# Deci-AI/super-gradients

Hardware: NVIDIA H100
Metric: images/sec YOLO-NAS-S 640 bf16 train (higher is better)
Workload: dtype bf16

## Files before the change

include/sgb200.h:

```cpp
#ifndef SGB200_H_
#define SGB200_H_

#include <stdint.h>

#ifdef __cplusplus
extern "C" {
#endif

#define SGB_OK 0
#define SGB_E_INVALID (-1)
#define SGB_E_UNSUPPORTED (-2)
#define SGB_E_CUDA (-3)
#define SGB_E_ARCH (-4)

#define SGB_ACT_NONE 0
#define SGB_ACT_RELU 1
#define SGB_ACT_SILU 2

typedef uint16_t sgb_bf16;

typedef struct SgbConvDesc {
  int32_t N, H, W, C;
  int32_t K, R, S;
  int32_t P, Q;
  int32_t stride, pad;
  int32_t x_pitch, x_off;
  int32_t y_pitch, y_off;
  int32_t up2;
  int32_t centre_from;
} SgbConvDesc;

typedef struct SgbEpilogue {
  const float* scale;
  const float* shift;
  const sgb_bf16* residual;
  double* stats;
  int32_t stats_repl;
  int32_t act;
  int32_t out_f32;
} SgbEpilogue;

const char* sgb_last_error(void);
int sgb_version(void);
int sgb_check_device(void);
int64_t sgb_sm100_launches(void);
int64_t sgb_conv_halo_launches(void);
void sgb_conv_force_im2col(int on);
int64_t sgb_conv_wgrad_halo_launches(void);
void sgb_conv_wgrad_force_im2col(int on);

int sgb_conv_fprop(const SgbConvDesc* d, const sgb_bf16* x, const sgb_bf16* w_krsc, void* y, const SgbEpilogue* ep,
                   void* stream);
int sgb_conv_dgrad(const SgbConvDesc* d, const sgb_bf16* dy, const sgb_bf16* w_crsk, sgb_bf16* dx, int accumulate,
                   void* stream);
int sgb_conv_wgrad(const SgbConvDesc* d, const sgb_bf16* x, const sgb_bf16* dy, float* dw_krsc, void* stream);
int sgb_weight_prepare(const float* w_oihw, int K, int C, int R, int S, int c_pad, sgb_bf16* w_krsc, sgb_bf16* w_crsk,
                       const float* scale, int add_identity, void* stream);
int sgb_wgrad_to_oihw(const float* dw_krsc, int K, int C, int R, int S, int c_pad, float* g_oihw, int accumulate,
                      void* stream);
typedef struct SgbWeightItem {
  const float* w;
  const float* scale;
  sgb_bf16* krsc;
  sgb_bf16* crsk;
  int32_t K, C, R, S, c_pad, add_identity;
  int32_t kp, koff, etaps, etap;
  int64_t start;
} SgbWeightItem;
typedef struct SgbWgradItem {
  const float* dw;
  float* g;
  int32_t K, C, R, S, c_pad, accumulate;
  int64_t start;
} SgbWgradItem;
int sgb_weight_prepare_batch(const SgbWeightItem* items_dev, int n_items, int64_t total, void* stream);
typedef struct SgbAlphaItem {
  const float* dw1;
  const float* w1;
  const float* alpha;
// ... 348 lines not shown
```

super_gradients_b200/csrc/capi.cu:

```cuda
#include <cstdarg>
#include <cstdio>

#include "common.cuh"
#include "conv_sm100.h"
#include "sm100_host.h"

static thread_local char g_err[512] = "";

void sgb_set_error(const char* fmt, ...) {
  va_list ap;
  va_start(ap, fmt);
  vsnprintf(g_err, sizeof(g_err), fmt, ap);
  va_end(ap);
}

int sgb_cuda_check(cudaError_t e, const char* what) {
  if (e == cudaSuccess) return SGB_OK;
  sgb_set_error("%s: %s", what, cudaGetErrorString(e));
  return SGB_E_CUDA;
}

extern "C" const char* sgb_last_error(void) { return g_err; }
extern "C" int sgb_version(void) { return 100; }
extern "C" int sgb_check_device(void) {
  int dev = 0;
  if (int rc = sgb_cuda_check(cudaGetDevice(&dev), "cudaGetDevice")) return rc;
  cudaDeviceProp prop;
  if (int rc = sgb_cuda_check(cudaGetDeviceProperties(&prop, dev), "cudaGetDeviceProperties")) return rc;
  if (prop.major != 9) {
    sgb_set_error("libsgb200 is built for sm_90a only; device is sm_%d%d", prop.major, prop.minor);
    return SGB_E_ARCH;
  }
  return SGB_OK;
}

extern "C" int64_t sgb_sm100_launches(void) { return (int64_t)sm100::launch_count(); }
extern "C" int64_t sgb_conv_halo_launches(void) { return (int64_t)sm100::halo_launch_count(); }
extern "C" void sgb_conv_force_im2col(int on) { sm100::force_im2col(on != 0); }
extern "C" int64_t sgb_conv_wgrad_halo_launches(void) { return (int64_t)sm100::wgrad_halo_launch_count(); }
extern "C" void sgb_conv_wgrad_force_im2col(int on) { sm100::wgrad_force_im2col(on != 0); }
```

super_gradients_b200/csrc/conv_sm100.cu:

```cuda
#include <cuda.h>

#include <cstdlib>
#include <cstring>

#include "common.cuh"
#include "conv_sm100.h"
#include "sm100_host.h"
#include "sm100_ptx.cuh"

namespace sm100 {

constexpr int BLOCK_M = 128;
constexpr int NUM_THREADS = 384;
constexpr int CONSUMER_THREADS = 256;
constexpr int MAX_STAGES = 8;

struct Params {
  int M;
  int N;
  int C;
  int KC;
  int n_tiles;
  int stages;
  int P, Q;
// ... 13 lines not shown
  int stats_repl;
  int act;
  int centre_n, centre_c;
};

template <int BN>
__device__ __forceinline__ int off_centre_steps(const Params& p, int nt, int steps, int step_ch) {
  if (p.centre_n > 0 && nt * BN >= p.centre_n) return 0;
  if (p.centre_c > 0) return (p.centre_c + step_ch - 1) / step_ch;
  return steps;
}
constexpr int CENTRE_TAP = 4;

__device__ __forceinline__ long long out_row(const Params& p, long long m) {
  if (p.out_mode == 0) return m;
  const int pq = p.P * p.Q;
  const int n = (int)(m / pq);
  const int rem = (int)(m - (long long)n * pq);
  const int j = rem / p.Q, i = rem - j * p.Q;
  return ((long long)n * p.outH + j * p.o_mul + p.oh_add) * p.outW + i * p.o_mul + p.ow_add;
}

__device__ __forceinline__ void consumer_sync() { asm volatile("bar.sync 1, %0;" ::"n"(CONSUMER_THREADS) : "memory"); }
template <int WARPS>
__device__ __forceinline__ void group_sync(int wg) {
  if (WARPS == 8)
    consumer_sync();
  else
    asm volatile("bar.sync %0, 128;" ::"r"(2 + wg) : "memory");
}

constexpr uint32_t CTRL_BAR_BYTES = 16u * MAX_STAGES;

template <int BN, int WARPS = 8>
__device__ __forceinline__ void tile_epilogue(const Params& p, const float (&acc)[BN / 2], const long long (&orow)[2],
                                              const bool (&row_ok)[2], int nt, int wg, int wq, int lane, float* s_part,
                                              float* s_stats) {
  const int n0 = nt * BN;
  const int ncols = min(BN, p.N - n0);
  bf16* yrow[2];
  const bf16* rrow[2];
#pragma unroll
  for (int h = 0; h < 2; ++h) {
    yrow[h] = p.y + orow[h] * p.y_pitch + p.y_off + n0;
    rrow[h] = p.residual ? p.residual + orow[h] * p.y_pitch + p.y_off + n0 : nullptr;
  }
#pragma unroll
  for (int j = 0; j < BN / 8; ++j) {
    const int col = 8 * j + 2 * (lane & 3);
    const bool col_ok = col < ncols;
    float sum0 = 0.f, sum1 = 0.f, sq0 = 0.f, sq1 = 0.f;
#pragma unroll
    for (int h = 0; h < 2; ++h) {
      float v0 = acc[4 * j + 2 * h], v1 = acc[4 * j + 2 * h + 1];
      const bool ok = row_ok[h] && col_ok;
      if (p.scale && col_ok) {
        v0 *= p.scale[n0 + col];
        v1 *= p.scale[n0 + col + 1];
      }
      if (p.shift && col_ok) {
        v0 += p.shift[n0 + col];
        v1 += p.shift[n0 + col + 1];
      }
      if (rrow[h] && ok) {
        const uint32_t rr = *reinterpret_cast<const uint32_t*>(rrow[h] + col);
        v0 += __uint_as_float(rr << 16);
        v1 += __uint_as_float(rr & 0xffff0000u);
      }
      if (p.act != SGB_ACT_NONE) {
        v0 = apply_act(v0, p.act);
        v1 = apply_act(v1, p.act);
      }
      __nv_bfloat162 hh = __floats2bfloat162_rn(v0, v1);
      const uint32_t pk = *reinterpret_cast<uint32_t*>(&hh);
      if (ok) {
        *reinterpret_cast<uint32_t*>(yrow[h] + col) = pk;
        const float lo = __uint_as_float(pk << 16), hi = __uint_as_float(pk & 0xffff0000u);
        sum0 += lo;
        sum1 += hi;
        sq0 = fmaf(lo, lo, sq0);
        sq1 = fmaf(hi, hi, sq1);
      }
    }
    if (p.stats) {
#pragma unroll
      for (int o = 4; o < 32; o <<= 1) {
        sum0 += __shfl_xor_sync(0xffffffffu, sum0, o);
        sum1 += __shfl_xor_sync(0xffffffffu, sum1, o);
        sq0 += __shfl_xor_sync(0xffffffffu, sq0, o);
        sq1 += __shfl_xor_sync(0xffffffffu, sq1, o);
      }
      if (lane < 4) {
        float* part = s_part + (WARPS == 8 ? wg * 4 + wq : wq) * 2 * BN;
        part[col] = sum0;
        part[col + 1] = sum1;
        part[BN + col] = sq0;
        part[BN + col + 1] = sq1;
      }
    }
  }
  if (p.stats) {
    group_sync<WARPS>(wg);
    for (int i = threadIdx.x - 128 - (WARPS == 8 ? 0 : 128 * wg); i < 2 * BN; i += WARPS * 32) {
      const int which = i / BN, c = i - which * BN;
      if (c < ncols) {
        float v = 0.f;
#pragma unroll
        for (int w = 0; w < WARPS; ++w) v += s_part[w * 2 * BN + i];
        s_stats[which * p.N + n0 + c] += v;
// ... 99 lines not shown
        wgmma_commit();
        if (prev >= 0) {
          wgmma_wait<1>();
          __syncwarp();
          if (lane == 0) mbar_arrive(empty_bar(prev));
        }
        prev = stg;
        if (++stg == p.stages) {
          stg = 0;
          par ^= 1;
        }
      }
      wgmma_wait<0>();
      fence_regs(acc);
      __syncwarp();
      if (lane == 0 && prev >= 0) mbar_arrive(empty_bar(prev));

      const long long m_lo = (long long)mt * BLOCK_M + wg * 64 + wq * 16 + (lane >> 2);
      long long orow[2];
      bool row_ok[2];
#pragma unroll
      for (int h = 0; h < 2; ++h) {
        const long long m = m_lo + 8 * h;
        row_ok[h] = m < p.M;
        orow[h] = out_row(p, row_ok[h] ? m : 0);
      }
      tile_epilogue<BN>(p, acc, orow, row_ok, nt, wg, wq, lane, s_part, s_stats);
    }
  }
  __syncthreads();
  flush_stats(p, s_stats);
}

constexpr int HALO_W = 10, HALO_H = 10, HALO_TILE = 8;
constexpr uint32_t HALO_CG_BYTES = 1664;
constexpr uint32_t HALO_CTRL_BYTES = CTRL_BAR_BYTES + 16;
constexpr int HALO_MAX_STAGES = 6;

template <int BN, bool SKIP>
__global__ void __launch_bounds__(NUM_THREADS, BN <= 48 ? 2 : 1)
conv3x3_halo_kernel(const __grid_constant__ CUtensorMap map_a, const __grid_constant__ CUtensorMap map_b, const Params p) {
  extern __shared__ __align__(1024) unsigned char smem_raw[];
  const uint32_t smem_base = (smem_u32(smem_raw) + 1023u) & ~1023u;
  const int ksteps = p.C / 16;
  constexpr uint32_t b_box = BN * 32;
  const uint32_t b_bytes = 9u * ksteps * b_box;
  const uint32_t a_stage = ((uint32_t)(p.C / 8) * HALO_CG_BYTES + 1023u) & ~1023u;
  const uint32_t sb = smem_base, sa0 = smem_base + ((b_bytes + 1023u) & ~1023u);
  const uint32_t ctrl = sa0 + p.stages * a_stage;
  auto full_bar = [&](int s) { return ctrl + 8u * s; };
  auto empty_bar = [&](int s) { return ctrl + 8u * (MAX_STAGES + s); };
  const uint32_t b_bar = ctrl + CTRL_BAR_BYTES;
  float* s_part = reinterpret_cast<float*>(smem_raw + (ctrl + HALO_CTRL_BYTES - smem_u32(smem_raw)));
  float* s_stats = s_part + 8 * 2 * BN;

  const int warp = threadIdx.x >> 5, lane = threadIdx.x & 31;
  const int m_tiles = p.M;
  const int nt = blockIdx.x % p.n_tiles;
  const int mt_step = gridDim.x / p.n_tiles;
  const int mt0 = blockIdx.x / p.n_tiles;
  const int off = SKIP ? off_centre_steps<BN>(p, nt, ksteps, 16) : ksteps;

  if (threadIdx.x == 0) {
    for (int s = 0; s < p.stages; ++s) {
      mbar_init(full_bar(s), 1);
      mbar_init(empty_bar(s), 4);
// ... 325 lines not shown
        mbar_wait(empty_bar(stg), par);
        const uint32_t sa = smem_base + stg * stage_bytes;
        mbar_expect_tx(full_bar(stg), tx);
        tma_load_tiled_4d(sa, &map_dy, full_bar(stg), 64 * rb, tw * HALO_TILE, th * HALO_TILE, n_img);
        for (int cg = 0; cg < NB / 8; ++cg)
          tma_load_tiled_4d(sa + a_bytes + (uint32_t)cg * HALO_CG_BYTES, &map_x, full_bar(stg), ctile * NB + 8 * cg,
                            tw * HALO_TILE - 1, th * HALO_TILE - 1, n_img);
        if (++stg == p.stages) {
          stg = 0;
          par ^= 1;
        }
      }
    }
  } else if (warp >= 4) {
    const int wg = (warp >> 2) - 1;
    const uint32_t ring = smem_base, bars = ctrl;
    if (!all_taps && wg == 0)
      wgrad_halo_consume<NB, 1>(p, ring, bars, t0, t1, CENTRE_TAP, rb, ctile);
    else if (!all_taps)
      wgrad_halo_consume<NB, 0>(p, ring, bars, t0, t1, 0, rb, ctile);
    else if (wg == 0)
      wgrad_halo_consume<NB, 5>(p, ring, bars, t0, t1, 0, rb, ctile);
    else
      wgrad_halo_consume<NB, 4>(p, ring, bars, t0, t1, 5, rb, ctile);
  }
}

EncodeTiledFn g_tiled = nullptr;
EncodeIm2colFn g_im2col = nullptr;
int g_num_sms = 0;
long long g_launches = 0;
long long g_halo_launches = 0;
long long g_wgrad_halo_launches = 0;
bool g_force_im2col = false;
bool g_wgrad_force_im2col = false;
long long launch_count() { return g_launches; }
long long halo_launch_count() { return g_halo_launches; }
long long wgrad_halo_launch_count() { return g_wgrad_halo_launches; }
void force_im2col(bool on) { g_force_im2col = on; }
void wgrad_force_im2col(bool on) { g_wgrad_force_im2col = on; }

int init_driver() {
  if (g_tiled && g_im2col) return SGB_OK;
  cudaDriverEntryPointQueryResult qres;
  void* fn = nullptr;
  if (cudaGetDriverEntryPoint("cuTensorMapEncodeTiled", &fn, cudaEnableDefault, &qres) != cudaSuccess || !fn) {
    sgb_set_error("cuTensorMapEncodeTiled entry point not found");
    return SGB_E_CUDA;
  }
  g_tiled = (EncodeTiledFn)fn;
  fn = nullptr;
  if (cudaGetDriverEntryPoint("cuTensorMapEncodeIm2col", &fn, cudaEnableDefault, &qres) != cudaSuccess || !fn) {
    sgb_set_error("cuTensorMapEncodeIm2col entry point not found");
    return SGB_E_CUDA;
  }
  g_im2col = (EncodeIm2colFn)fn;
  int dev = 0;
  cudaGetDevice(&dev);
  cudaDeviceGetAttribute(&g_num_sms, cudaDevAttrMultiProcessorCount, dev);
  return SGB_OK;
}

CUtensorMapSwizzle swizzle_for(int kc) {
  return kc == 64 ? CU_TENSOR_MAP_SWIZZLE_128B : (kc == 32 ? CU_TENSOR_MAP_SWIZZLE_64B : CU_TENSOR_MAP_SWIZZLE_32B);
}

bool supported(const Problem& q) {
  if (q.C % 16 != 0 || q.b_rows % 8 != 0) return false;
  if (!((q.R == 1 && q.S == 1) || (q.R == 3 && q.S == 3))) return false;
  if (q.stride != 1 && q.stride != 2) return false;
  if (q.a_pitch % 8 != 0 || q.y_pitch % 8 != 0 || q.y_off % 8 != 0) return false;
  if (((uintptr_t)q.a & 15) || ((uintptr_t)q.b & 15) || ((uintptr_t)q.y & 15)) return false;
  if ((long long)q.N * q.P * q.Q >= (1ll << 31)) return false;
  if (q.b_rows > 4096) return false;
  return true;
}

namespace {

template <class Fn>
struct Variant {
  int bn;
  Fn fn;
  int regs;
  bool ready;
};
typedef void (*ConvFn)(const CUtensorMap, const CUtensorMap, const Params);
typedef void (*WgradFn)(const CUtensorMap, const CUtensorMap, const WParams);
Variant<ConvFn> g_conv[] = {{16, conv_wgmma_kernel<16, false>, 0, false},   {32, conv_wgmma_kernel<32, false>, 0, false},
                            {48, conv_wgmma_kernel<48, false>, 0, false},   {64, conv_wgmma_kernel<64, false>, 0, false},
                            {96, conv_wgmma_kernel<96, false>, 0, false},   {128, conv_wgmma_kernel<128, false>, 0, false}};
Variant<ConvFn> g_conv_skip[] = {{16, conv_wgmma_kernel<16, true>, 0, false},   {32, conv_wgmma_kernel<32, true>, 0, false},
                                 {48, conv_wgmma_kernel<48, true>, 0, false},   {64, conv_wgmma_kernel<64, true>, 0, false},
                                 {96, conv_wgmma_kernel<96, true>, 0, false},   {128, conv_wgmma_kernel<128, true>, 0, false}};
Variant<ConvFn> g_halo[] = {{16, conv3x3_halo_kernel<16, false>, 0, false},   {32, conv3x3_halo_kernel<32, false>, 0, false},
                            {48, conv3x3_halo_kernel<48, false>, 0, false},   {64, conv3x3_halo_kernel<64, false>, 0, false},
                            {96, conv3x3_halo_kernel<96, false>, 0, false},   {128, conv3x3_halo_kernel<128, false>, 0, false}};
Variant<ConvFn> g_halo_skip[] = {{16, conv3x3_halo_kernel<16, true>, 0, false},   {32, conv3x3_halo_kernel<32, true>, 0, false},
                                 {48, conv3x3_halo_kernel<48, true>, 0, false},   {64, conv3x3_halo_kernel<64, true>, 0, false},
                                 {96, conv3x3_halo_kernel<96, true>, 0, false},   {128, conv3x3_halo_kernel<128, true>, 0, false}};
Variant<WgradFn> g_wgrad[] = {{16, wgrad_wgmma_kernel<16>, 0, false}, {32, wgrad_wgmma_kernel<32>, 0, false},
                              {48, wgrad_wgmma_kernel<48>, 0, false}, {64, wgrad_wgmma_kernel<64>, 0, false},
                              {96, wgrad_wgmma_kernel<96>, 0, false}, {128, wgrad_wgmma_kernel<128>, 0, false}};
Variant<WgradFn> g_wgrad_halo[] = {{16, wgrad3x3_halo_kernel<16>, 0, false}, {32, wgrad3x3_halo_kernel<32>, 0, false},
                                   {48, wgrad3x3_halo_kernel<48>, 0, false}};

template <class Fn>
int prepare(Variant<Fn>& v, const char* what) {
  if (v.ready) return SGB_OK;
  if (int rc = sgb_cuda_check(cudaFuncSetAttribute(v.fn, cudaFuncAttributeMaxDynamicSharedMemorySize, 227 * 1024), what)) return rc;
  cudaFuncAttributes fa{};
  if (int rc = sgb_cuda_check(cudaFuncGetAttributes(&fa, v.fn), what)) return rc;
  v.regs = fa.numRegs;
  v.ready = true;
  return SGB_OK;
}

int pick_bn(int n) {
  for (int bn : {16, 32, 48, 64, 96, 128})
    if (n <= bn) return bn;
  int best = 128, best_waste = (n + 127) / 128 * 128 - n;
  for (int bn : {96, 64}) {
    const int waste = (n + bn - 1) / bn * bn - n;
    if (waste < best_waste) { best_waste = waste; best = bn; }
  }
  return best;
}

size_t halo_smem(int C, int bn, int n, bool stats, int stages) {
  const size_t b_bytes = ((size_t)9 * C * bn * 2 + 1023) & ~(size_t)1023;
  const size_t a_stage = ((size_t)(C / 8) * HALO_CG_BYTES + 1023) & ~(size_t)1023;
  return 1024 + b_bytes + (size_t)stages * a_stage + HALO_CTRL_BYTES + (stats ? (size_t)(8 * 2 * bn + 4 * n) * 4 : 0);
}
// ... 48 lines not shown
  int stages = 0;
  for (;; --ctas_per_sm) {
    const size_t budget = (ctas_per_sm == 1 ? 227u : 227u / ctas_per_sm - 1u) * 1024u;
    for (stages = HALO_MAX_STAGES; stages >= 2 && halo_smem(q.C, bn, p.N, p.stats != nullptr, stages) > budget; --stages) {
    }
    if (stages >= 2 || ctas_per_sm == 1) break;
  }
  if (stages < 2) { sgb_set_error("conv3x3_halo: tile does not fit shared memory"); return SGB_E_UNSUPPORTED; }
  p.stages = stages;
  const size_t smem = halo_smem(q.C, bn, p.N, p.stats != nullptr, stages);

  alignas(64) CUtensorMap map_a, map_b;
  if (int rc = encode_halo_map(&map_a, q.a, q.N, q.H, q.W, q.C, q.a_pitch)) return rc;
  {
    cuuint64_t dims[2] = {(cuuint64_t)q.b_cols, (cuuint64_t)q.b_rows};
    cuuint64_t strides[1] = {(cuuint64_t)q.b_cols * 2};
    cuuint32_t box[2] = {16, (cuuint32_t)bn};
    cuuint32_t estr[2] = {1, 1};
    CUresult r = g_tiled(&map_b, CU_TENSOR_MAP_DATA_TYPE_BFLOAT16, 2, const_cast<void*>(q.b), dims, strides, box, estr,
                         CU_TENSOR_MAP_INTERLEAVE_NONE, CU_TENSOR_MAP_SWIZZLE_32B, CU_TENSOR_MAP_L2_PROMOTION_L2_128B,
                         CU_TENSOR_MAP_FLOAT_OOB_FILL_NONE);
    if (r != CUDA_SUCCESS) {
      sgb_set_error("cuTensorMapEncodeTiled(halo B) failed with %d (cols=%d rows=%d BN=%d)", (int)r, q.b_cols, q.b_rows, bn);
      return SGB_E_CUDA;
    }
  }
  int per_nt = g_num_sms * ctas_per_sm / p.n_tiles;
  if (per_nt > p.M) per_nt = p.M;
  if (per_nt < 1) per_nt = 1;
  var->fn<<<per_nt * p.n_tiles, NUM_THREADS, smem, st>>>(map_a, map_b, p);
  ++g_launches;
  ++g_halo_launches;
  return sgb_cuda_check(cudaGetLastError(), "conv3x3_halo_kernel");
}

}

int launch(const Problem& q, cudaStream_t st) {
  if (int rc = init_driver()) return rc;
  Params p{};
  p.M = q.N * q.P * q.Q;
  p.N = q.b_rows;
  p.C = q.C;
  p.KC = q.C % 64 == 0 ? 64 : (q.C % 32 == 0 ? 32 : 16);
  if (p.KC < 64 && q.C > 32) p.KC = 64;
  const int bn = pick_bn(p.N);
  p.n_tiles = (p.N + bn - 1) / bn;
  p.P = q.P; p.Q = q.Q; p.stride = q.stride; p.pad = q.pad;
  if (q.ntaps > 0) {
    p.ntaps = q.ntaps;
    for (int t = 0; t < q.ntaps; ++t) { p.tap_dh[t] = (signed char)q.tap_dh[t]; p.tap_dw[t] = (signed char)q.tap_dw[t]; p.tap_b[t] = (signed char)q.tap_b[t]; }
  } else {
    p.ntaps = q.R * q.S;
    for (int t = 0; t < p.ntaps; ++t) {
      p.tap_dh[t] = (signed char)(t / q.S);
      p.tap_dw[t] = (signed char)(t % q.S);
      p.tap_b[t] = (signed char)(q.flip ? (p.ntaps - 1 - t) : t);
    }
  }
  if (p.ntaps > 9) return SGB_E_UNSUPPORTED;
  p.out_mode = q.out_mode; p.o_mul = q.o_mul; p.oh_add = q.oh_add; p.ow_add = q.ow_add; p.outH = q.outH; p.outW = q.outW;
  p.b_cols_per_tap = q.b_cols_per_tap;
  p.y = (bf16*)q.y; p.y_pitch = q.y_pitch; p.y_off = q.y_off;
  p.scale = q.scale; p.shift = q.shift; p.residual = (const bf16*)q.residual;
  p.stats = q.stats; p.stats_repl = q.stats_repl > 0 ? q.stats_repl : 1; p.act = q.act;
  if (q.centre_from > 0) {
    if (q.R != 3 || q.S != 3 || q.stride != 1 || q.pad != 1 || q.ntaps > 0 || q.centre_from % 16 != 0 ||
        q.centre_from >= (q.flip ? q.C : q.b_rows))
      return SGB_E_INVALID;
    (q.flip ? p.centre_c : p.centre_n) = q.centre_from;
  }
  if (!g_force_im2col)
    if (const int hbn = halo_bn(q)) return launch_halo(q, p, hbn, st);
  Variant<ConvFn>* var = nullptr;
  for (auto& v : p.centre_n > 0 || p.centre_c > 0 ? g_conv_skip : g_conv)
    if (v.bn == bn) var = &v;
  if (int rc = prepare(*var, "conv_wgmma_kernel")) return rc;
  const uint32_t a_bytes = BLOCK_M * p.KC * 2, b_bytes = ((uint32_t)(bn * p.KC * 2) + 1023u) & ~1023u;
  const uint32_t stage_bytes = a_bytes + b_bytes;
  const uint32_t ctrl_bytes = CTRL_BAR_BYTES + (p.stats ? (uint32_t)(8 * 2 * bn + 2 * p.N) * 4u : 0u);
  const int regs_alloc = ((var->regs + 7) / 8) * 8 * NUM_THREADS;
  int ctas_per_sm = 65536 / regs_alloc;
  if (ctas_per_sm > 2) ctas_per_sm = 2;
  if (ctas_per_sm < 1) ctas_per_sm = 1;
  int stages = 0;
  for (;; --ctas_per_sm) {
    const uint32_t budget = (ctas_per_sm == 1 ? 226u : 227u / ctas_per_sm - 1u) * 1024u;
    stages = budget > ctrl_bytes + 1024 ? (int)((budget - ctrl_bytes - 1024) / stage_bytes) : 0;
    if (stages > MAX_STAGES) stages = MAX_STAGES;
    if (stages >= 4 || ctas_per_sm == 1) break;
  }
  if (stages < 2) { sgb_set_error("conv_wgmma: tile does not fit shared memory"); return SGB_E_UNSUPPORTED; }
  p.stages = stages;
  const size_t smem = 1024 + (size_t)stages * stage_bytes + ctrl_bytes;

  alignas(64) CUtensorMap map_a, map_b;
  {
    cuuint64_t dims[4] = {(cuuint64_t)q.C, (cuuint64_t)q.W, (cuuint64_t)q.H, (cuuint64_t)q.N};
    cuuint64_t strides[3] = {(cuuint64_t)q.a_pitch * 2, (cuuint64_t)q.W * q.a_pitch * 2, (cuuint64_t)q.H * q.W * q.a_pitch * 2};
    int lower[2] = {-q.pad, -q.pad};
    int upper[2] = {q.pad - (q.S - 1), q.pad - (q.R - 1)};
    if (q.ntaps > 0) {
      lower[0] = lower[1] = 0;
      upper[0] = q.Q - q.W;
      upper[1] = q.P - q.H;
    }
// ... 166 lines not shown
```

super_gradients_b200/csrc/conv_sm100.h:

```cpp
#pragma once
#include <cuda_runtime.h>

namespace sm100 {

struct Problem {
  const void* a;
  int N, H, W, C, a_pitch;
  const void* b;
  int b_rows, b_cols, b_cols_per_tap;
  int R, S, stride, pad, P, Q, flip;
  int ntaps;
  int tap_dh[9], tap_dw[9], tap_b[9];
  int out_mode, o_mul, oh_add, ow_add, outH, outW;
  void* y;
  int y_pitch, y_off;
  const float* scale;
  const float* shift;
  const void* residual;
  double* stats;
  int stats_repl, act;
  int centre_from;
};

struct WgradProblem {
  const void* x;
  const void* dy;
  int N, H, W, C, x_pitch;
  int K, y_pitch;
  int R, S, stride, pad, P, Q;
  float* dw;
  int centre_from;
};

bool wgrad_supported(const WgradProblem& q);
int wgrad_launch(const WgradProblem& q, cudaStream_t st);
bool supported(const Problem& q);
int launch(const Problem& q, cudaStream_t st);
long long launch_count();
long long halo_launch_count();
void force_im2col(bool on);
long long wgrad_halo_launch_count();
void wgrad_force_im2col(bool on);

}
```

super_gradients_b200/csrc/sm100_ptx.cuh:

```cuda
#pragma once
#include <cuda.h>

#include "common.cuh"

namespace sm100 {

__device__ __forceinline__ void mbar_init(uint32_t bar, uint32_t count) {
  asm volatile("mbarrier.init.shared::cta.b64 [%0], %1;" ::"r"(bar), "r"(count));
}
__device__ __forceinline__ void mbar_expect_tx(uint32_t bar, uint32_t bytes) {
  asm volatile("mbarrier.arrive.expect_tx.shared::cta.b64 _, [%0], %1;" ::"r"(bar), "r"(bytes) : "memory");
}
__device__ __forceinline__ void mbar_arrive(uint32_t bar) {
  asm volatile("mbarrier.arrive.shared::cta.b64 _, [%0];" ::"r"(bar) : "memory");
}
__device__ __forceinline__ void mbar_wait(uint32_t bar, uint32_t parity) {
  asm volatile(
      "{\n"
      ".reg .pred p;\n"
      "WAIT_LOOP:\n"
      "mbarrier.try_wait.parity.shared::cta.b64 p, [%0], %1;\n"
      "@p bra DONE;\n"
      "bra WAIT_LOOP;\n"
      "DONE:\n"
// ... 127 lines not shown
  asm volatile(
      "{\n.reg .pred p;\nsetp.ne.b32 p, %66, 0;\n"
      "wgmma.mma_async.sync.aligned.m64n128k16.f32.bf16.bf16 {%0,%1,%2,%3,%4,%5,%6,%7,%8,%9,%10,%11,%12,%13,%14,%15,%16,%17,%18,%19,%20,%21,%22,%23,%24,%25,%26,%27,%28,%29,%30,%31,%32,%33,%34,%35,%36,%37,%38,%39,%40,%41,%42,%43,%44,%45,%46,%47,%48,%49,%50,%51,%52,%53,%54,%55,%56,%57,%58,%59,%60,%61,%62,%63}, %64, %65, p, 1, 1, 0, 0;\n}\n"
      : "+f"(d[0]), "+f"(d[1]), "+f"(d[2]), "+f"(d[3]), "+f"(d[4]), "+f"(d[5]), "+f"(d[6]), "+f"(d[7]), "+f"(d[8]), "+f"(d[9]), "+f"(d[10]), "+f"(d[11]), "+f"(d[12]), "+f"(d[13]), "+f"(d[14]), "+f"(d[15]), "+f"(d[16]), "+f"(d[17]), "+f"(d[18]), "+f"(d[19]), "+f"(d[20]), "+f"(d[21]), "+f"(d[22]), "+f"(d[23]), "+f"(d[24]), "+f"(d[25]), "+f"(d[26]), "+f"(d[27]), "+f"(d[28]), "+f"(d[29]), "+f"(d[30]), "+f"(d[31]), "+f"(d[32]), "+f"(d[33]), "+f"(d[34]), "+f"(d[35]), "+f"(d[36]), "+f"(d[37]), "+f"(d[38]), "+f"(d[39]), "+f"(d[40]), "+f"(d[41]), "+f"(d[42]), "+f"(d[43]), "+f"(d[44]), "+f"(d[45]), "+f"(d[46]), "+f"(d[47]), "+f"(d[48]), "+f"(d[49]), "+f"(d[50]), "+f"(d[51]), "+f"(d[52]), "+f"(d[53]), "+f"(d[54]), "+f"(d[55]), "+f"(d[56]), "+f"(d[57]), "+f"(d[58]), "+f"(d[59]), "+f"(d[60]), "+f"(d[61]), "+f"(d[62]), "+f"(d[63])
      : "l"(da), "l"(db), "r"(accumulate));
}
template <>
__device__ __forceinline__ void mma_mn<128>(float (&d)[64], uint64_t da, uint64_t db, uint32_t accumulate) {
  asm volatile(
      "{\n.reg .pred p;\nsetp.ne.b32 p, %66, 0;\n"
      "wgmma.mma_async.sync.aligned.m64n128k16.f32.bf16.bf16 {%0,%1,%2,%3,%4,%5,%6,%7,%8,%9,%10,%11,%12,%13,%14,%15,%16,%17,%18,%19,%20,%21,%22,%23,%24,%25,%26,%27,%28,%29,%30,%31,%32,%33,%34,%35,%36,%37,%38,%39,%40,%41,%42,%43,%44,%45,%46,%47,%48,%49,%50,%51,%52,%53,%54,%55,%56,%57,%58,%59,%60,%61,%62,%63}, %64, %65, p, 1, 1, 1, 1;\n}\n"
      : "+f"(d[0]), "+f"(d[1]), "+f"(d[2]), "+f"(d[3]), "+f"(d[4]), "+f"(d[5]), "+f"(d[6]), "+f"(d[7]), "+f"(d[8]), "+f"(d[9]), "+f"(d[10]), "+f"(d[11]), "+f"(d[12]), "+f"(d[13]), "+f"(d[14]), "+f"(d[15]), "+f"(d[16]), "+f"(d[17]), "+f"(d[18]), "+f"(d[19]), "+f"(d[20]), "+f"(d[21]), "+f"(d[22]), "+f"(d[23]), "+f"(d[24]), "+f"(d[25]), "+f"(d[26]), "+f"(d[27]), "+f"(d[28]), "+f"(d[29]), "+f"(d[30]), "+f"(d[31]), "+f"(d[32]), "+f"(d[33]), "+f"(d[34]), "+f"(d[35]), "+f"(d[36]), "+f"(d[37]), "+f"(d[38]), "+f"(d[39]), "+f"(d[40]), "+f"(d[41]), "+f"(d[42]), "+f"(d[43]), "+f"(d[44]), "+f"(d[45]), "+f"(d[46]), "+f"(d[47]), "+f"(d[48]), "+f"(d[49]), "+f"(d[50]), "+f"(d[51]), "+f"(d[52]), "+f"(d[53]), "+f"(d[54]), "+f"(d[55]), "+f"(d[56]), "+f"(d[57]), "+f"(d[58]), "+f"(d[59]), "+f"(d[60]), "+f"(d[61]), "+f"(d[62]), "+f"(d[63])
      : "l"(da), "l"(db), "r"(accumulate));
}


__device__ __forceinline__ uint64_t smem_desc(uint32_t smem_addr, int row_bytes, uint32_t lbo_bytes, uint32_t sbo_bytes) {
  const uint64_t layout = row_bytes == 128 ? 1u : (row_bytes == 64 ? 2u : 3u);
  return (uint64_t)((smem_addr >> 4) & 0x3fff) | ((uint64_t)((lbo_bytes >> 4) & 0x3fff) << 16) |
         ((uint64_t)((sbo_bytes >> 4) & 0x3fff) << 32) | (layout << 62);
}
__device__ __forceinline__ uint64_t smem_desc_noswizzle(uint32_t smem_addr, uint32_t lbo_bytes, uint32_t sbo_bytes) {
  return (uint64_t)((smem_addr >> 4) & 0x3fff) | ((uint64_t)((lbo_bytes >> 4) & 0x3fff) << 16) |
         ((uint64_t)((sbo_bytes >> 4) & 0x3fff) << 32);
}

__device__ __forceinline__ void tma_load_tiled_4d(uint32_t dst, const CUtensorMap* map, uint32_t bar, int c0, int c1, int c2, int c3) {
  asm volatile(
      "cp.async.bulk.tensor.4d.shared::cluster.global.mbarrier::complete_tx::bytes [%0], [%1, {%3, %4, %5, %6}], [%2];" ::"r"(dst),
      "l"(reinterpret_cast<uint64_t>(map)), "r"(bar), "r"(c0), "r"(c1), "r"(c2), "r"(c3)
      : "memory");
}

}
```

super_gradients_b200/lib.py:

```python
import ctypes
import os
from ctypes import POINTER, Structure, c_char_p, c_double, c_float, c_int, c_int32, c_int64, c_void_p

_HERE = os.path.dirname(os.path.abspath(__file__))
LIB_PATH = os.path.join(_HERE, "libsgb200.so")

ACT_NONE, ACT_RELU, ACT_SILU = 0, 1, 2


class SgbError(RuntimeError):
    pass


class ConvDesc(Structure):
    _fields_ = [(n, c_int32) for n in ("N", "H", "W", "C", "K", "R", "S", "P", "Q", "stride", "pad", "x_pitch", "x_off", "y_pitch", "y_off", "up2", "centre_from")]


class Epilogue(Structure):
    _fields_ = [
        ("scale", c_void_p),
        ("shift", c_void_p),
        ("residual", c_void_p),
        ("stats", c_void_p),
        ("stats_repl", c_int32),
# ... 100 lines not shown
        ("alpha", c_float),
        ("beta", c_float),
        ("w_cls", c_float),
        ("w_iou", c_float),
        ("w_dfl", c_float),
        ("iou_type", c_int32),
    ]


class NmsDesc(Structure):
    _fields_ = [
        ("B", c_int32),
        ("L", c_int32),
        ("ncls", c_int32),
        ("score_thr", c_float),
        ("iou_thr", c_double),
        ("top_k", c_int32),
        ("max_out", c_int32),
        ("multi_label", c_int32),
        ("class_agnostic", c_int32),
        ("thr_inclusive", c_int32),
    ]


P = c_void_p
_I, _F, _L = c_int, c_float, c_int64

_SIGNATURES = {
    "sgb_last_error": (c_char_p, []),
    "sgb_version": (c_int, []),
    "sgb_check_device": (c_int, []),
    "sgb_sm100_launches": (c_int64, []),
    "sgb_conv_halo_launches": (c_int64, []),
    "sgb_conv_force_im2col": (None, [_I]),
    "sgb_conv_wgrad_halo_launches": (c_int64, []),
    "sgb_conv_wgrad_force_im2col": (None, [_I]),
    "sgb_conv_fprop": (c_int, [POINTER(ConvDesc), P, P, P, POINTER(Epilogue), P]),
    "sgb_conv_dgrad": (c_int, [POINTER(ConvDesc), P, P, P, _I, P]),
    "sgb_conv_wgrad": (c_int, [POINTER(ConvDesc), P, P, P, P]),
    "sgb_weight_prepare": (c_int, [P, _I, _I, _I, _I, _I, P, P, P, _I, P]),
    "sgb_wgrad_to_oihw": (c_int, [P, _I, _I, _I, _I, _I, P, _I, P]),
    "sgb_weight_prepare_batch": (c_int, [P, _I, c_int64, P]),
    "sgb_wgrad_to_oihw_batch": (c_int, [P, _I, c_int64, P]),
    "sgb_qarep_alpha_finish_batch": (c_int, [P, _I, P]),
    "sgb_convt2x2_fprop": (c_int, [POINTER(ConvDesc), P, P, P, P, P]),
    "sgb_nchw_f32_to_nhwc_bf16": (c_int, [P, _I, _I, _I, _I, P, _I, _I, _I, P]),
    "sgb_stem_patches_f32": (c_int, [P, _I, _I, _I, _I, _I, _I, _I, P, _I, _I, _I, P]),
    "sgb_nhwc_bf16_to_nchw_f32": (c_int, [P, _I, _I, _I, _I, _I, _I, P, P]),
    "sgb_bn_act_fwd": (c_int, [POINTER(BnDesc), P, P, P, P, P, P, P, P, P, P, P]),
    "sgb_bn_act_fwd_fused": (c_int, [POINTER(BnDesc), P, P, P, P, P, P, P, P, P, P, P]),
    "sgb_bn_act_infer": (c_int, [POINTER(BnDesc), P, P, P, P, P, P, P, P]),
    "sgb_bn_act_bwd_reduce": (c_int, [POINTER(BnDesc), P, P, P, P, P, P, P, P, P]),
    "sgb_bn_act_bwd_apply": (c_int, [POINTER(BnDesc), P, P, P, P, P, P, P, P, P, P, P, P, P]),
    "sgb_bn_act_bwd_fused": (c_int, [POINTER(BnDesc), P, P, P, P, P, P, P, P, P, P, P, P, P]),
    "sgb_channel_stats": (c_int, [P, _L, _I, _I, _I, P, P]),
    "sgb_qarep_moments": (c_int, [POINTER(QarepDesc), P, P, P, P]),
    "sgb_qarep_fwd": (c_int, [POINTER(QarepDesc)] + [P] * 15),
    "sgb_qarep_fwd_fused": (c_int, [POINTER(QarepDesc)] + [P] * 15),
    "sgb_qarep_bwd_reduce": (c_int, [POINTER(QarepDesc), P, P, P, P, P, P, P]),
    "sgb_qarep_bwd_apply": (c_int, [POINTER(QarepDesc)] + [P] * 16),
    "sgb_qarep_bwd_fused": (c_int, [POINTER(QarepDesc)] + [P] * 15),
    "sgb_maxpool_fwd": (c_int, [P, _I, _I, _I, _I, _I, _I, _I, _I, _I, P, _I, _I, _I, _I, P, P]),
    "sgb_maxpool_bwd": (c_int, [P, _I, _I, _I, _I, _I, _I, _I, _I, _I, _I, _I, P, P, P]),
    "sgb_maxpool_bwd_bf16": (c_int, [P, _I, _I, _I, _I, _I, _I, _I, _I, _I, _I, _I, P, P, _I, P]),
    "sgb_axpby": (c_int, [P, _I, _I, _F, P, _I, _I, _F, P, _I, _I, _L, _I, P]),
    "sgb_scale_add": (c_int, [P, _I, _I, P, P, _I, _I, P, _I, _I, _L, _I, P]),
# ... 6 lines not shown
    "sgb_pose_keypoint_decode": (c_int, [P, _I, P, _I, _I, _I, _I, _I, _I, _I, _I, _F, _F, _F, _I, P, P, P, P]),
    "sgb_tal_assign": (c_int, [POINTER(LossDesc)] + [P] * 12 + [_L, P]),
    "sgb_tal_workspace_bytes": (c_int64, [POINTER(LossDesc)]),
    "sgb_atss_assign": (c_int, [POINTER(LossDesc)] + [P] * 5 + [c_int32] + [P] * 7 + [P, _L, P]),
    "sgb_atss_workspace_bytes": (c_int64, [POINTER(LossDesc)]),
    "sgb_dfl_iou_loss_fwd_bwd": (c_int, [POINTER(LossDesc)] + [P] * 8 + [_F, P, P, P]),
    "sgb_focal_cls_fwd_bwd": (c_int, [POINTER(LossDesc), P, P, P, P, c_float, c_float, P, P]),
    "sgb_loss_finalize": (c_int, [POINTER(LossDesc), P, P, P]),
    "sgb_preprocess_u8": (c_int, [POINTER(PreprocDesc), P, P, P]),
    "sgb_resample_crop_u8": (c_int, [P, P, P, _L, _I, _I, _I, _I, _I, _I, c_double, P, P, P, P]),
    "sgb_classify_rows": (c_int, [P, _L, _I, _L, _I, P, P, _L, _I, _I, P, P, P, P]),
    "sgb_detection_augment": (c_int, [P, P, P, _L, _I, _I, _I, _I, _I, _I, c_double, _I, P, P]),
    "sgb_pose_augment": (c_int, [P, P, P, _L, P, _L, _I, _I, _I, c_double, _I, P, P]),
    "sgb_detection_matching": (c_int, [POINTER(MatchDesc), P, P, P, P, P, P, P, P, P, P]),
    "sgb_pose_keypoint_matching": (c_int, [P] * 10 + [_I] * 6 + [P] * 7),
    "sgb_pose_tal_workspace_bytes": (c_int64, [POINTER(PoseLossDesc)]),
    "sgb_pose_tal_assign": (c_int, [POINTER(PoseLossDesc)] + [P] * 14 + [_L, P]),
    "sgb_pose_loss_fwd_bwd": (c_int, [POINTER(PoseLossDesc)] + [P] * 12 + [_F] + [P] * 5),
    "sgb_pose_loss_finalize": (c_int, [POINTER(PoseLossDesc), P, P, P]),
    "sgb_head_grad_scatter": (c_int, [P, _I, _I, _I, _I, _I, P, _I, P]),
    "sgb_sliding_window_gather": (c_int, [P, _I, _I, _I, _I, P, P, _I, _I, P, P]),
    "sgb_sliding_window_merge_workspace_bytes": (c_int64, [_I, P, _I, _I, _I]),
    "sgb_sliding_window_merge": (c_int, [P, P, P, P, P, _I, _I, _I, _I, c_double, P, P, P, _L, P]),
    "sgb_sliding_window_merge_launches": (c_int32, [_I, P, _I, _I]),
    "sgb_nms_workspace_bytes": (c_int64, [POINTER(NmsDesc)]),
    "sgb_batched_nms": (c_int, [POINTER(NmsDesc), P, P, P, P, P, P, _L, P]),
    "sgb_sgd_step": (c_int, [P, P, P, _L, P, P]),
    "sgb_adamw_step": (c_int, [P, P, P, P, _L, P, P]),
    "sgb_ema_update": (c_int, [P, P, _L, P, P]),
}

_lib = None

LAUNCH_COUNT = {"sgb_tal_assign": 4, "sgb_atss_assign": 3, "sgb_pose_tal_assign": 4, "sgb_sm100_launches": 0, "sgb_conv_halo_launches": 0, "sgb_conv_force_im2col": 0, "sgb_conv_wgrad_halo_launches": 0, "sgb_conv_wgrad_force_im2col": 0, "sgb_sliding_window_merge_workspace_bytes": 0, "sgb_sliding_window_merge_launches": 0, "sgb_last_error": 0, "sgb_version": 0, "sgb_check_device": 0}
LAUNCHES = [0]


def exported_names():
    return sorted(_SIGNATURES)


def load():
    global _lib
    if _lib is not None:
        return _lib
    if not os.path.exists(LIB_PATH):
        raise SgbError(f"{LIB_PATH} not found: run `python -c 'import __graft_entry__ as g; g.build()'` " "(there is no non-CUDA fallback for this package)")
    lib = ctypes.CDLL(LIB_PATH)
    for name, (res, args) in _SIGNATURES.items():
        fn = getattr(lib, name)
        fn.restype = res
        fn.argtypes = args
    _lib = lib
    return lib


def check(rc, what=""):
    if rc != 0:
        msg = load().sgb_last_error()
        raise SgbError(f"{what} failed with code {rc}: {msg.decode() if msg else ''}")


def call(name, *args):
    lib = load()
    rc = getattr(lib, name)(*args)
    LAUNCHES[0] += LAUNCH_COUNT.get(name, 1)
    if rc != 0:
# ... 3 lines not shown
```

Baseline: 957.7.

## Add persistent 1x1 conv kernel with resident filters and TMA-store epilogue

Adds a dedicated persistent kernel for stride-1, unpadded 1x1 convolutions. Each CTA loads its full filter slice into shared memory once, then streams activation tiles through a TMA pipeline over many M tiles. The output is staged in shared memory and written back with bulk TMA stores. The aim is to remove repeated filter reloads and uncoalesced per-thread stores from the im2col path. It is only taken when the filter fits in shared memory and there are enough tile rounds, and it adds shared-memory pressure and extra barrier syncs in the epilogue.

```diff
diff --git a/include/sgb200.h b/include/sgb200.h
--- a/include/sgb200.h
+++ b/include/sgb200.h
@@ -45,6 +45,7 @@
 int sgb_check_device(void);
 int64_t sgb_sm100_launches(void);
 int64_t sgb_conv_halo_launches(void);
+int64_t sgb_conv_1x1_launches(void);
 void sgb_conv_force_im2col(int on);
 int64_t sgb_conv_wgrad_halo_launches(void);
 void sgb_conv_wgrad_force_im2col(int on);
diff --git a/super_gradients_b200/csrc/capi.cu b/super_gradients_b200/csrc/capi.cu
--- a/super_gradients_b200/csrc/capi.cu
+++ b/super_gradients_b200/csrc/capi.cu
@@ -36,6 +36,7 @@
 
 extern "C" int64_t sgb_sm100_launches(void) { return (int64_t)sm100::launch_count(); }
 extern "C" int64_t sgb_conv_halo_launches(void) { return (int64_t)sm100::halo_launch_count(); }
+extern "C" int64_t sgb_conv_1x1_launches(void) { return (int64_t)sm100::conv1x1_launch_count(); }
 extern "C" void sgb_conv_force_im2col(int on) { sm100::force_im2col(on != 0); }
 extern "C" int64_t sgb_conv_wgrad_halo_launches(void) { return (int64_t)sm100::wgrad_halo_launch_count(); }
 extern "C" void sgb_conv_wgrad_force_im2col(int on) { sm100::wgrad_force_im2col(on != 0); }
diff --git a/super_gradients_b200/csrc/conv_sm100.cu b/super_gradients_b200/csrc/conv_sm100.cu
--- a/super_gradients_b200/csrc/conv_sm100.cu
+++ b/super_gradients_b200/csrc/conv_sm100.cu
@@ -69,10 +69,10 @@
 
 constexpr uint32_t CTRL_BAR_BYTES = 16u * MAX_STAGES;
 
-template <int BN, int WARPS = 8>
+template <int BN, int WARPS = 8, bool STAGED = false>
 __device__ __forceinline__ void tile_epilogue(const Params& p, const float (&acc)[BN / 2], const long long (&orow)[2],
                                               const bool (&row_ok)[2], int nt, int wg, int wq, int lane, float* s_part,
-                                              float* s_stats) {
+                                              float* s_stats, uint32_t* s_tile = nullptr) {
   const int n0 = nt * BN;
   const int ncols = min(BN, p.N - n0);
   bf16* yrow[2];
@@ -110,8 +110,9 @@
       }
       __nv_bfloat162 hh = __floats2bfloat162_rn(v0, v1);
       const uint32_t pk = *reinterpret_cast<uint32_t*>(&hh);
+      if (STAGED) s_tile[(wq * 16 + (lane >> 2) + 8 * h) * (BN / 2) + col / 2] = pk;
       if (ok) {
-        *reinterpret_cast<uint32_t*>(yrow[h] + col) = pk;
+        if (!STAGED) *reinterpret_cast<uint32_t*>(yrow[h] + col) = pk;
         const float lo = __uint_as_float(pk << 16), hi = __uint_as_float(pk & 0xffff0000u);
         sum0 += lo;
         sum1 += hi;
@@ -277,6 +278,130 @@
   flush_stats(p, s_stats);
 }
 
+constexpr uint32_t C1_CTRL_BYTES = CTRL_BAR_BYTES + 16;
+
+__host__ __device__ constexpr uint32_t c1_chunk_bytes(int bn, int kc) { return ((uint32_t)(bn * kc * 2) + 1023u) & ~1023u; }
+
+template <int BN>
+__global__ void __launch_bounds__(NUM_THREADS, 1)
+conv1x1_kernel(const __grid_constant__ CUtensorMap map_a, const __grid_constant__ CUtensorMap map_b,
+               const __grid_constant__ CUtensorMap map_y, const Params p) {
+  extern __shared__ __align__(1024) unsigned char smem_raw[];
+  const uint32_t smem_base = (smem_u32(smem_raw) + 1023u) & ~1023u;
+  const int chunks = (p.C + p.KC - 1) / p.KC;
+  const uint32_t a_bytes = BLOCK_M * p.KC * 2, b_chunk = c1_chunk_bytes(BN, p.KC);
+  const uint32_t sb = smem_base, sa0 = smem_base + (uint32_t)chunks * b_chunk;
+  const uint32_t s_out = sa0 + p.stages * a_bytes;
+  const uint32_t ctrl = s_out + 2u * 64u * BN * 2u;
+  auto full_bar = [&](int s) { return ctrl + 8u * s; };
+  auto empty_bar = [&](int s) { return ctrl + 8u * (MAX_STAGES + s); };
+  const uint32_t b_bar = ctrl + CTRL_BAR_BYTES;
+  float* s_part = reinterpret_cast<float*>(smem_raw + (ctrl + C1_CTRL_BYTES - smem_u32(smem_raw)));
+  float* s_stats = s_part + 8 * 2 * BN;
+
+  const int warp = threadIdx.x >> 5, lane = threadIdx.x & 31;
+  const int m_tiles = (p.M + BLOCK_M - 1) / BLOCK_M;
+  const int nt = blockIdx.x % p.n_tiles;
+  const int mt_step = gridDim.x / p.n_tiles;
+  const int mt0 = blockIdx.x / p.n_tiles;
+
+  if (threadIdx.x == 0) {
+    for (int s = 0; s < p.stages; ++s) {
+      mbar_init(full_bar(s), 1);
+      mbar_init(empty_bar(s), 8);
+    }
+    mbar_init(b_bar, 1);
+    asm volatile("fence.mbarrier_init.release.cluster;" ::: "memory");
+    asm volatile("fence.proxy.async.shared::cta;" ::: "memory");
+  }
+  if (p.stats)
+    for (int i = threadIdx.x; i < 2 * p.N; i += NUM_THREADS) s_stats[i] = 0.f;
+  __syncthreads();
+
+  if (warp == 0) {
+    if (elect_one()) {
+      mbar_expect_tx(b_bar, (uint32_t)chunks * BN * p.KC * 2);
+      for (int ck = 0; ck < chunks; ++ck) tma_load_2d(sb + (uint32_t)ck * b_chunk, &map_b, b_bar, ck * p.KC, nt * BN);
+      int stg = 0;
+      uint32_t par = 1;
+      for (int mt = mt0; mt < m_tiles; mt += mt_step) {
+        for (int ck = 0; ck < chunks; ++ck) {
+          mbar_wait(empty_bar(stg), par);
+          const uint32_t sa = sa0 + stg * a_bytes;
+          mbar_expect_tx(full_bar(stg), a_bytes);
+          tma_load_2d(sa, &map_a, full_bar(stg), ck * p.KC, mt * BLOCK_M);
+          if (++stg == p.stages) {
+            stg = 0;
+            par ^= 1;
+          }
+        }
+      }
+    }
+  } else if (warp >= 4) {
+    const int wg = (warp >> 2) - 1;
+    const int wq = warp & 3;
+    const int row_bytes = p.KC * 2;
+    const uint32_t sbo = 8u * (uint32_t)row_bytes;
+    const int ksteps = p.KC / 16;
+    float acc[BN / 2];
+    int stg = 0;
+    uint32_t par = 0;
+    mbar_wait(b_bar, 0);
+    for (int mt = mt0; mt < m_tiles; mt += mt_step) {
+      int prev = -1;
+      for (int k = 0; k < chunks; ++k) {
+        mbar_wait(full_bar(stg), par);
+        const uint32_t sa_wg = sa0 + stg * a_bytes + (uint32_t)wg * 64u * (uint32_t)row_bytes, sb_k = sb + (uint32_t)k * b_chunk;
+        wgmma_fence();
+        for (int j = 0; j < ksteps; ++j) {
+          const uint64_t da = smem_desc(sa_wg + 32u * j, row_bytes, 16u, sbo), db = smem_desc(sb_k + 32u * j, row_bytes, 16u, sbo);
+          mma_kk<BN>(acc, da, db, (k | j) != 0);
+        }
+        wgmma_commit();
+        if (prev >= 0) {
+          wgmma_wait<1>();
+          __syncwarp();
+          if (lane == 0) mbar_arrive(empty_bar(prev));
+        }
+        prev = stg;
+        if (++stg == p.stages) {
+          stg = 0;
+          par ^= 1;
+        }
+      }
+      wgmma_wait<0>();
+      fence_regs(acc);
+      __syncwarp();
+      if (lane == 0) mbar_arrive(empty_bar(prev));
+
+      const long long m_lo = (long long)mt * BLOCK_M + wg * 64 + wq * 16 + (lane >> 2);
+      long long orow[2];
+      bool row_ok[2];
+#pragma unroll
+      for (int h = 0; h < 2; ++h) {
+        const long long m = m_lo + 8 * h;
+        row_ok[h] = m < p.M;
+        orow[h] = row_ok[h] ? m : 0;
+      }
+      const bool leader = wq == 0 && lane == 0;
+      const uint32_t s_tile = s_out + (uint32_t)wg * 64u * BN * 2u;
+      if (leader) bulk_wait_read();
+      group_sync<4>(wg);
+      tile_epilogue<BN, 8, true>(p, acc, orow, row_ok, nt, wg, wq, lane, s_part, s_stats,
+                                 reinterpret_cast<uint32_t*>(smem_raw + (s_tile - smem_u32(smem_raw))));
+      fence_proxy_async();
+      group_sync<4>(wg);
+      if (leader) {
+        tma_store_2d(&map_y, s_tile, nt * BN, mt * BLOCK_M + wg * 64);
+        bulk_commit();
+      }
+    }
+    if (wq == 0 && lane == 0) bulk_wait();
+  }
+  __syncthreads();
+  flush_stats(p, s_stats);
+}
+
 constexpr int HALO_W = 10, HALO_H = 10, HALO_TILE = 8;
 constexpr uint32_t HALO_CG_BYTES = 1664;
 constexpr uint32_t HALO_CTRL_BYTES = CTRL_BAR_BYTES + 16;
@@ -668,10 +793,12 @@
 long long g_launches = 0;
 long long g_halo_launches = 0;
 long long g_wgrad_halo_launches = 0;
+long long g_conv1x1_launches = 0;
 bool g_force_im2col = false;
 bool g_wgrad_force_im2col = false;
 long long launch_count() { return g_launches; }
 long long halo_launch_count() { return g_halo_launches; }
+long long conv1x1_launch_count() { return g_conv1x1_launches; }
 long long wgrad_halo_launch_count() { return g_wgrad_halo_launches; }
 void force_im2col(bool on) { g_force_im2col = on; }
 void wgrad_force_im2col(bool on) { g_wgrad_force_im2col = on; }
@@ -735,6 +862,10 @@
 Variant<ConvFn> g_halo_skip[] = {{16, conv3x3_halo_kernel<16, true>, 0, false},   {32, conv3x3_halo_kernel<32, true>, 0, false},
                                  {48, conv3x3_halo_kernel<48, true>, 0, false},   {64, conv3x3_halo_kernel<64, true>, 0, false},
                                  {96, conv3x3_halo_kernel<96, true>, 0, false},   {128, conv3x3_halo_kernel<128, true>, 0, false}};
+typedef void (*Conv1x1Fn)(const CUtensorMap, const CUtensorMap, const CUtensorMap, const Params);
+Variant<Conv1x1Fn> g_conv1x1[] = {{16, conv1x1_kernel<16>, 0, false}, {32, conv1x1_kernel<32>, 0, false},
+                               {48, conv1x1_kernel<48>, 0, false}, {64, conv1x1_kernel<64>, 0, false},
+                               {96, conv1x1_kernel<96>, 0, false}, {128, conv1x1_kernel<128>, 0, false}};
 Variant<WgradFn> g_wgrad[] = {{16, wgrad_wgmma_kernel<16>, 0, false}, {32, wgrad_wgmma_kernel<32>, 0, false},
                               {48, wgrad_wgmma_kernel<48>, 0, false}, {64, wgrad_wgmma_kernel<64>, 0, false},
                               {96, wgrad_wgmma_kernel<96>, 0, false}, {128, wgrad_wgmma_kernel<128>, 0, false}};
@@ -849,6 +980,96 @@
   ++g_launches;
   ++g_halo_launches;
   return sgb_cuda_check(cudaGetLastError(), "conv3x3_halo_kernel");
+}
+
+size_t conv1x1_smem(int C, int kc, int bn, int n, bool stats, int stages) {
+  const size_t chunks = (size_t)(C + kc - 1) / kc;
+  return 1024 + chunks * c1_chunk_bytes(bn, kc) + (size_t)stages * BLOCK_M * kc * 2 + (size_t)2 * 64 * bn * 2 + C1_CTRL_BYTES +
+         (stats ? (size_t)(8 * 2 * bn + 2 * n) * 4 : 0);
+}
+
+bool conv1x1_takes(const Problem& q, int kc, int bn) {
+  if (q.R != 1 || q.S != 1 || q.stride != 1 || q.pad != 0 || q.ntaps > 0 || q.out_mode != 0) return false;
+  if (q.P != q.H || q.Q != q.W) return false;
+  if (conv1x1_smem(q.C, kc, bn, q.b_rows, q.stats != nullptr, 6) > 226 * 1024) return false;
+  const long long m_tiles = ((long long)q.N * q.P * q.Q + BLOCK_M - 1) / BLOCK_M, n_tiles = (q.b_rows + bn - 1) / bn;
+  const long long rounds = (m_tiles * n_tiles + g_num_sms - 1) / g_num_sms;
+  long long per_nt = g_num_sms / n_tiles;
+  if (per_nt > m_tiles) per_nt = m_tiles;
+  if (per_nt < 1) per_nt = 1;
+  return rounds >= 6 && (m_tiles + per_nt - 1) / per_nt <= rounds;
+}
+
+int launch_conv1x1(const Problem& q, const Params& p0, int bn, cudaStream_t st) {
+  Params p = p0;
+  Variant<Conv1x1Fn>* var = nullptr;
+  for (auto& v : g_conv1x1)
+    if (v.bn == bn) var = &v;
+  if (int rc = prepare(*var, "conv1x1_kernel")) return rc;
+  const int regs_alloc = ((var->regs + 7) / 8) * 8 * NUM_THREADS;
+  int ctas_per_sm = 65536 / regs_alloc;
+  if (ctas_per_sm > 2) ctas_per_sm = 2;
+  if (ctas_per_sm < 1) ctas_per_sm = 1;
+  const size_t fixed = conv1x1_smem(q.C, p.KC, bn, p.N, p.stats != nullptr, 0), a_bytes = (size_t)BLOCK_M * p.KC * 2;
+  int stages = 0;
+  for (;; --ctas_per_sm) {
+    const size_t budget = (ctas_per_sm == 1 ? 226u : 227u / ctas_per_sm - 1u) * 1024u;
+    stages = budget > fixed ? (int)((budget - fixed) / a_bytes) : 0;
+    if (stages > MAX_STAGES) stages = MAX_STAGES;
+    if (stages >= 4 || ctas_per_sm == 1) break;
+  }
+  if (stages < 4) { sgb_set_error("conv1x1: filter slice does not fit shared memory"); return SGB_E_UNSUPPORTED; }
+  p.stages = stages;
+  const size_t smem = fixed + (size_t)stages * a_bytes;
+
+  alignas(64) CUtensorMap map_a, map_b, map_y;
+  {
+    cuuint64_t dims[2] = {(cuuint64_t)q.C, (cuuint64_t)p.M};
+    cuuint64_t strides[1] = {(cuuint64_t)q.a_pitch * 2};
+    cuuint32_t box[2] = {(cuuint32_t)p.KC, (cuuint32_t)BLOCK_M};
+    cuuint32_t estr[2] = {1, 1};
+    CUresult r = g_tiled(&map_a, CU_TENSOR_MAP_DATA_TYPE_BFLOAT16, 2, const_cast<void*>(q.a), dims, strides, box, estr,
+                         CU_TENSOR_MAP_INTERLEAVE_NONE, swizzle_for(p.KC), CU_TENSOR_MAP_L2_PROMOTION_L2_128B,
+                         CU_TENSOR_MAP_FLOAT_OOB_FILL_NONE);
+    if (r != CUDA_SUCCESS) {
+      sgb_set_error("cuTensorMapEncodeTiled(1x1 A) failed with %d (C=%d M=%d pitch=%d KC=%d)", (int)r, q.C, p.M, q.a_pitch, p.KC);
+      return SGB_E_CUDA;
+    }
+  }
+  {
+    cuuint64_t dims[2] = {(cuuint64_t)q.b_cols, (cuuint64_t)q.b_rows};
+    cuuint64_t strides[1] = {(cuuint64_t)q.b_cols * 2};
+    cuuint32_t box[2] = {(cuuint32_t)p.KC, (cuuint32_t)bn};
+    cuuint32_t estr[2] = {1, 1};
+    CUresult r = g_tiled(&map_b, CU_TENSOR_MAP_DATA_TYPE_BFLOAT16, 2, const_cast<void*>(q.b), dims, strides, box, estr,
+                         CU_TENSOR_MAP_INTERLEAVE_NONE, swizzle_for(p.KC), CU_TENSOR_MAP_L2_PROMOTION_L2_128B,
+                         CU_TENSOR_MAP_FLOAT_OOB_FILL_NONE);
+    if (r != CUDA_SUCCESS) {
+      sgb_set_error("cuTensorMapEncodeTiled(1x1 B) failed with %d (cols=%d rows=%d KC=%d BN=%d)", (int)r, q.b_cols, q.b_rows, p.KC, bn);
+      return SGB_E_CUDA;
+    }
+  }
+  {
+    cuuint64_t dims[2] = {(cuuint64_t)p.N, (cuuint64_t)p.M};
+    cuuint64_t strides[1] = {(cuuint64_t)q.y_pitch * 2};
+    cuuint32_t box[2] = {(cuuint32_t)bn, 64};
+    cuuint32_t estr[2] = {1, 1};
+    CUresult r = g_tiled(&map_y, CU_TENSOR_MAP_DATA_TYPE_BFLOAT16, 2, (bf16*)q.y + q.y_off, dims, strides, box, estr,
+                         CU_TENSOR_MAP_INTERLEAVE_NONE, CU_TENSOR_MAP_SWIZZLE_NONE, CU_TENSOR_MAP_L2_PROMOTION_L2_128B,
+                         CU_TENSOR_MAP_FLOAT_OOB_FILL_NONE);
+    if (r != CUDA_SUCCESS) {
+      sgb_set_error("cuTensorMapEncodeTiled(1x1 y) failed with %d (N=%d M=%d pitch=%d BN=%d)", (int)r, p.N, p.M, q.y_pitch, bn);
+      return SGB_E_CUDA;
+    }
+  }
+  const int m_tiles = (p.M + BLOCK_M - 1) / BLOCK_M;
+  int per_nt = g_num_sms * ctas_per_sm / p.n_tiles;
+  if (per_nt > m_tiles) per_nt = m_tiles;
+  if (per_nt < 1) per_nt = 1;
+  var->fn<<<per_nt * p.n_tiles, NUM_THREADS, smem, st>>>(map_a, map_b, map_y, p);
+  ++g_launches;
+  ++g_conv1x1_launches;
+  return sgb_cuda_check(cudaGetLastError(), "conv1x1_kernel");
 }
 
 }
@@ -887,8 +1108,10 @@
       return SGB_E_INVALID;
     (q.flip ? p.centre_c : p.centre_n) = q.centre_from;
   }
-  if (!g_force_im2col)
+  if (!g_force_im2col) {
     if (const int hbn = halo_bn(q)) return launch_halo(q, p, hbn, st);
+    if (conv1x1_takes(q, p.KC, bn)) return launch_conv1x1(q, p, bn, st);
+  }
   Variant<ConvFn>* var = nullptr;
   for (auto& v : p.centre_n > 0 || p.centre_c > 0 ? g_conv_skip : g_conv)
     if (v.bn == bn) var = &v;
diff --git a/super_gradients_b200/csrc/conv_sm100.h b/super_gradients_b200/csrc/conv_sm100.h
--- a/super_gradients_b200/csrc/conv_sm100.h
+++ b/super_gradients_b200/csrc/conv_sm100.h
@@ -38,6 +38,7 @@
 int launch(const Problem& q, cudaStream_t st);
 long long launch_count();
 long long halo_launch_count();
+long long conv1x1_launch_count();
 void force_im2col(bool on);
 long long wgrad_halo_launch_count();
 void wgrad_force_im2col(bool on);
diff --git a/super_gradients_b200/csrc/sm100_ptx.cuh b/super_gradients_b200/csrc/sm100_ptx.cuh
--- a/super_gradients_b200/csrc/sm100_ptx.cuh
+++ b/super_gradients_b200/csrc/sm100_ptx.cuh
@@ -183,4 +183,14 @@
       : "memory");
 }
 
+__device__ __forceinline__ void tma_store_2d(const CUtensorMap* map, uint32_t src, int c0, int c1) {
+  asm volatile("cp.async.bulk.tensor.2d.global.shared::cta.bulk_group [%0, {%2, %3}], [%1];" ::"l"(reinterpret_cast<uint64_t>(map)),
+               "r"(src), "r"(c0), "r"(c1)
+               : "memory");
 }
+__device__ __forceinline__ void bulk_commit() { asm volatile("cp.async.bulk.commit_group;" ::: "memory"); }
+__device__ __forceinline__ void bulk_wait_read() { asm volatile("cp.async.bulk.wait_group.read 0;" ::: "memory"); }
+__device__ __forceinline__ void bulk_wait() { asm volatile("cp.async.bulk.wait_group 0;" ::: "memory"); }
+__device__ __forceinline__ void fence_proxy_async() { asm volatile("fence.proxy.async.shared::cta;" ::: "memory"); }
+
+}
diff --git a/super_gradients_b200/lib.py b/super_gradients_b200/lib.py
--- a/super_gradients_b200/lib.py
+++ b/super_gradients_b200/lib.py
@@ -156,6 +156,7 @@
     "sgb_check_device": (c_int, []),
     "sgb_sm100_launches": (c_int64, []),
     "sgb_conv_halo_launches": (c_int64, []),
+    "sgb_conv_1x1_launches": (c_int64, []),
     "sgb_conv_force_im2col": (None, [_I]),
     "sgb_conv_wgrad_halo_launches": (c_int64, []),
     "sgb_conv_wgrad_force_im2col": (None, [_I]),
@@ -228,7 +229,7 @@
 
 _lib = None
 
-LAUNCH_COUNT = {"sgb_tal_assign": 4, "sgb_atss_assign": 3, "sgb_pose_tal_assign": 4, "sgb_sm100_launches": 0, "sgb_conv_halo_launches": 0, "sgb_conv_force_im2col": 0, "sgb_conv_wgrad_halo_launches": 0, "sgb_conv_wgrad_force_im2col": 0, "sgb_sliding_window_merge_workspace_bytes": 0, "sgb_sliding_window_merge_launches": 0, "sgb_last_error": 0, "sgb_version": 0, "sgb_check_device": 0}
+LAUNCH_COUNT = {"sgb_tal_assign": 4, "sgb_atss_assign": 3, "sgb_pose_tal_assign": 4, "sgb_sm100_launches": 0, "sgb_conv_halo_launches": 0, "sgb_conv_1x1_launches": 0, "sgb_conv_force_im2col": 0, "sgb_conv_wgrad_halo_launches": 0, "sgb_conv_wgrad_force_im2col": 0, "sgb_sliding_window_merge_workspace_bytes": 0, "sgb_sliding_window_merge_launches": 0, "sgb_last_error": 0, "sgb_version": 0, "sgb_check_device": 0}
 LAUNCHES = [0]
 
 
```

Result: faster. 970.2, median of 6 (+1.3%).
